# ygtxr1997/MSML

Hardware: AMD Instinct MI355X
Metric: images/sec (112x112) ires50-MSML+PartialFC training step (higher is better)
Workload: dtype bf16; 1 GPU; iresnet50-MSML (OSB r18 + FM x4) + 85742-id ArcFace PartialFC, 112x112, batch 256/GPU, fwd+bwd+clip+SGD; global_batch=256, parallelism=dp1+class-parallel head, launch=eager, weight gradients + OSB on side streams

## Files before the change

msml_amd/csrc/wgrad_halo.hip:

```cpp
#include <stdlib.h>

#include <type_traits>

#include <mutex>

#include "common.h"
#include "options.h"

typedef __attribute__((ext_vector_type(4))) short s16x4;
typedef __attribute__((ext_vector_type(8))) short s16x8;
typedef __attribute__((address_space(3))) void* lptr_t;

#define WH_OOB 0x78000000u

typedef __attribute__((ext_vector_type(4))) unsigned int wh_rsrc_t;
__device__ __forceinline__ void wh_dma16(const wh_rsrc_t& rs, unsigned int lds, unsigned int off) {
#if defined(__HIP_DEVICE_COMPILE__)
  unsigned int keep;
  asm volatile("s_mov_b32 %0, m0\n\ts_mov_b32 m0, %3\n\ts_nop 0\n\tbuffer_load_dwordx4 %1, %2, 0 offen lds\n\ts_mov_b32 m0, %0"
               : "=&s"(keep)
               : "v"(off), "s"(rs), "s"(lds)
               : "memory");
#endif
}
__device__ __forceinline__ void wh_dma_wait() {
#if defined(__HIP_DEVICE_COMPILE__)
  asm volatile("s_waitcnt vmcnt(0)" ::: "memory");
#endif
}

#define WH_MAXGROUP 8
struct WgradHaloArgs {
  const unsigned short* u[WH_MAXGROUP]; int up; unsigned int u_bytes;
  const unsigned short* v[WH_MAXGROUP]; int vp; unsigned int v_bytes;
  int N, H, W, spy, spx;
  int XH, XW;
  int nstrips, chunk;
  int zper;
  int remap;
  int pair7;
  float* ws;
  BnIn xin;
};

template <int CO, bool XF = false, bool P7 = false>
__global__ void __launch_bounds__(512) __attribute__((amdgpu_waves_per_eu(2, 2))) k_wgrad_halo(const WgradHaloArgs p) {
#if defined(__HIP_DEVICE_COMPILE__)
  constexpr int NXB = 20;
  constexpr int GU = CO / 32, NI = CO / 64, UBLK = 7 * GU, NBLK = UBLK + NXB, NISS = (NBLK + 7) / 8;
  constexpr int UB = UBLK * 1024, VB = NXB * 1024, STAGE = UB + VB;
  extern __shared__ __attribute__((aligned(16))) char smem[];
  MSML_LDS_REGION(smem, 2 * STAGE + (XF ? 3 * 64 * 4 : 0));
  const int t = threadIdx.x, lane = t & 63;
  const int wave = __builtin_amdgcn_readfirstlane(t >> 6);
  constexpr bool R9 = CO == 128;
  const int mp = R9 ? (wave & 3) : (wave & 1), nh = R9 ? (wave >> 2) : ((wave >> 1) & 1), tg = R9 ? 0 : (wave >> 2);
  int bx = blockIdx.x, by = blockIdx.y, bz = blockIdx.z;
  if (p.remap) {
    const int T = gridDim.x * gridDim.y, total = T * gridDim.z;
    const int L = bx + gridDim.x * (by + gridDim.y * bz);
    const int Lp = (L & 7) * (total >> 3) + (L >> 3);
    const int tile = Lp % T;
    bz = Lp / T;
    bx = tile % gridDim.x;
    by = tile / gridDim.x;
  }
  const int layer = __builtin_amdgcn_readfirstlane(bz / p.zper);
  const int a0 = bx * CO, b0 = by * 64, split = bz - layer * p.zper;
  const int s_begin = split * p.chunk;
  int s_end = s_begin + p.chunk;
  if (s_end > p.nstrips) s_end = p.nstrips;
  const int spi = p.spy * p.spx;

  auto make_rsrc = [](const void* ptr, unsigned int bytes) -> wh_rsrc_t {
    const unsigned long long a = (unsigned long long)ptr;
    wh_rsrc_t r;
    r[0] = __builtin_amdgcn_readfirstlane((unsigned int)a);
    r[1] = __builtin_amdgcn_readfirstlane((unsigned int)(a >> 32) & 0xffffu);
    r[2] = __builtin_amdgcn_readfirstlane(bytes);
    r[3] = 0x00020000u;
    return r;
  };
  const wh_rsrc_t rs_u = make_rsrc(p.u[layer], p.u_bytes), rs_v = make_rsrc(p.v[layer], p.v_bytes);
  const unsigned int lds0 = __builtin_amdgcn_readfirstlane((unsigned int)(size_t)(lptr_t)smem);
  auto dma = [&](const wh_rsrc_t& rs, const char* dst, unsigned int off) {
    wh_dma16(rs, lds0 + (unsigned int)__builtin_amdgcn_readfirstlane((int)(dst - smem)), off);
  };

  const int lp = lane >> 2, lc = lane & 3;
  auto issue = [&](int strip, int buf) {
    char* ub = smem + buf * STAGE;
    char* vb = ub + UB;
    if constexpr (P7) {
      const int n = 2 * strip + (lp >> 3), x = lp & 7;
      const bool img = n < p.N;
#pragma unroll
      for (int i = 0; i < NISS; i++) {
        const int blk = wave + 8 * i;
        if (blk >= NBLK) break;
        if (blk < UBLK) {
          const int j = blk / GU, g = blk % GU;
          const unsigned int off = (img & (x < 7)) ? (unsigned int)((n * 7 + j) * 7 + x) * (unsigned int)(p.up * 2) +
                                                         (unsigned int)(a0 + g * 32 + lc * 8) * 2u
                                                   : WH_OOB;
          dma(rs_u, ub + blk * 1024, off);
        } else {
          const int bb = blk - UBLK, hr = bb >> 1, g = bb & 1;
          const int y = hr - 1;
          const bool ok = img & ((unsigned)y < 7u) & (x > 0);
          const unsigned int off = ok ? (unsigned int)((n * 7 + y) * 7 + x - 1) * (unsigned int)(p.vp * 2) +
                                            (unsigned int)(b0 + g * 32 + lc * 8) * 2u
                                      : WH_OOB;
          dma(rs_v, vb + bb * 1024, off);
        }
      }
      return;
    }
    const int n = strip / spi, rem = strip - n * spi, sy = rem / p.spx;
    const int y0 = sy * 7, x0 = (rem - sy * p.spx) * 14;
#pragma unroll
    for (int i = 0; i < NISS; i++) {
      const int blk = wave + 8 * i;
      if (blk >= NBLK) break;
      if (blk < UBLK) {
        const int j = blk / GU, g = blk % GU;
        const int y = y0 + j, x = x0 + lp;
        const bool ok = (lp < 14) & (x < p.W) & (y < p.H);
        const unsigned int off = ok ? (unsigned int)((n * p.H + y) * p.W + x) * (unsigned int)(p.up * 2) +
                                          (unsigned int)(a0 + g * 32 + lc * 8) * 2u
                                    : WH_OOB;
        dma(rs_u, ub + blk * 1024, off);
      } else {
        const int bb = blk - UBLK, hr = bb >> 1, g = bb & 1;
        const int y = y0 + hr - 1, x = x0 + lp - 1;
        const bool ok = (hr < 9) & ((unsigned)y < (unsigned)p.H) & ((unsigned)x < (unsigned)p.W);
        const unsigned int off = ok ? (unsigned int)((n * p.H + y) * p.W + x) * (unsigned int)(p.vp * 2) +
                                          (unsigned int)(b0 + g * 32 + lc * 8) * 2u
                                    : WH_OOB;
        dma(rs_v, vb + bb * 1024, off);
      }
    }
  };

  float* xtab = reinterpret_cast<float*>(smem + 2 * STAGE);
  auto xform = [&](int strip, int buf) {
    const int n = strip / spi, rem = strip - n * spi, sy = rem / p.spx;
    const int y0 = sy * 7, x0 = (rem - sy * p.spx) * 14;
    char* vb = smem + buf * STAGE + UB;
    const bool has_alpha = p.xin.alpha != nullptr;
#pragma unroll
    for (int i = 0; i < NISS; i++) {
      const int blk = wave + 8 * i;
      if (blk >= NBLK) break;
      if (blk >= UBLK) {
        const int bb = blk - UBLK, hr = bb >> 1, g = bb & 1;
        const int y = y0 + hr - 1, x = x0 + lp - 1;
        if ((hr < 9) & ((unsigned)y < (unsigned)p.H) & ((unsigned)x < (unsigned)p.W))
          bn_in_chunk(vb + bb * 1024 + lane * 16, xtab, 64, g * 32 + lc * 8, has_alpha);
      }
    }
  };

  constexpr int NA = R9 ? 1 : NI, NK = R9 ? 9 : 5;
  f32x16 acc[NA][NK];
#pragma unroll
  for (int i = 0; i < NA; i++)
#pragma unroll
    for (int k = 0; k < NK; k++)
#pragma unroll
      for (int e = 0; e < 16; e++) acc[i][k][e] = 0.f;

  const int g4 = lane >> 4, i16 = lane & 15, q4 = i16 >> 2, pp = i16 & 3;
  const int px = 8 * (g4 >> 1) + q4;
  const int chan = (2 * (g4 & 1) + (pp >> 1)) * 16 + (pp & 1) * 8;
  const int aofs = mp * NA * 1024 + px * 64 + chan;
  int vlo[3], vhi[3];
#pragma unroll
  for (int s = 0; s < 3; s++) {
    const int p0 = px + s, p1 = px + 4 + s;
    vlo[s] = nh * 1024 + (p0 >> 4) * 2048 + (p0 & 15) * 64 + chan;
    vhi[s] = nh * 1024 + (p1 >> 4) * 2048 + (p1 & 15) * 64 + chan;
  }
  const int ntaps = R9 ? 9 : (tg == 0 ? 5 : 4), tap0 = tg * 5;
  int vlok[5], vhik[5];
#pragma unroll
  for (int k = 0; k < 5; k++) {
    const int tp = tap0 + k, r = tp / 3, sft = tp - r * 3;
    vlok[k] = r * 2048 + (sft == 0 ? vlo[0] : (sft == 1 ? vlo[1] : vlo[2]));
    vhik[k] = r * 2048 + (sft == 0 ? vhi[0] : (sft == 1 ? vhi[1] : vhi[2]));
  }
  typedef __attribute__((address_space(3))) s16x4* tr_ptr;
  auto tr2 = [&](const char* lo, const char* hi) -> s16x8 {
    s16x4 l = __builtin_amdgcn_ds_read_tr16_b64_v4i16((tr_ptr)(lo));
    s16x4 h = __builtin_amdgcn_ds_read_tr16_b64_v4i16((tr_ptr)(hi));
    s16x8 o;
    o[0] = l[0]; o[1] = l[1]; o[2] = l[2]; o[3] = l[3];
    o[4] = h[0]; o[5] = h[1]; o[6] = h[2]; o[7] = h[3];
    return o;
  };

  if (s_begin < s_end) issue(s_begin, 0);
  if (XF) bn_in_fill(p.xin, xtab, b0, 64, t, 512);
  wh_dma_wait();
  __syncthreads();
  if (XF) {
    if (s_begin < s_end) xform(s_begin, 0);
    __syncthreads();
  }
  int cur = 0;
  s16x8 fa[2][NA], fb5[2][5], xr[4][3];
  for (int strip = s_begin; strip < s_end; strip++) {
    if (strip + 1 < s_end) issue(strip + 1, cur ^ 1);
    const char* ub = smem + cur * STAGE + aofs;
    const char* vb = smem + cur * STAGE + UB;
    if constexpr (R9) {
      auto fetch_a = [&](int j) { fa[j & 1][0] = tr2(ub + j * (GU * 1024), ub + j * (GU * 1024) + 256); };
      auto fetch_x = [&](int row) {
#pragma unroll
        for (int sft = 0; sft < 3; sft++) xr[row & 3][sft] = tr2(vb + row * 2048 + vlo[sft], vb + row * 2048 + vhi[sft]);
      };
      fetch_a(0);
      fetch_x(0);
      fetch_x(1);
      fetch_x(2);
#pragma unroll
      for (int j = 0; j < 7; j++) {
        if (j + 1 < 7) {
          fetch_a(j + 1);
          fetch_x(j + 3);
        }
        __builtin_amdgcn_sched_barrier(0);
#pragma unroll
        for (int k = 0; k < 9; k++)
          acc[0][k] = __builtin_amdgcn_mfma_f32_32x32x16_bf16(__builtin_bit_cast(bf16x8, fa[j & 1][0]),
                                                              __builtin_bit_cast(bf16x8, xr[(j + k / 3) & 3][k % 3]),
                                                              acc[0][k], 0, 0, 0);
        __builtin_amdgcn_sched_barrier(0);
        if (XF && j == 6 && strip + 1 < s_end) {
          wh_dma_wait();
          xform(strip + 1, cur ^ 1);
        }
      }
      wh_dma_wait();
      __syncthreads();
      cur ^= 1;
      continue;
    }
    auto fetch = [&](int j, int fb) {
#pragma unroll
      for (int i = 0; i < NA; i++)
        fa[fb][i] = tr2(ub + j * (GU * 1024) + i * 1024, ub + j * (GU * 1024) + i * 1024 + 256);
#pragma unroll
      for (int k = 0; k < 5; k++)
        if (k < ntaps) fb5[fb][k] = tr2(vb + j * 2048 + vlok[k], vb + j * 2048 + vhik[k]);
    };
    fetch(0, 0);
#pragma unroll
    for (int j = 0; j < 7; j++) {
      const int fb = j & 1;
      if (j + 1 < 7) fetch(j + 1, fb ^ 1);
      __builtin_amdgcn_sched_barrier(0);
#pragma unroll
      for (int k = 0; k < 5; k++)
        if (k < ntaps) {
#pragma unroll
          for (int i = 0; i < NA; i++)
            acc[i][k] = __builtin_amdgcn_mfma_f32_32x32x16_bf16(__builtin_bit_cast(bf16x8, fa[fb][i]),
                                                                __builtin_bit_cast(bf16x8, fb5[fb][k]), acc[i][k], 0, 0, 0);
        }
      __builtin_amdgcn_sched_barrier(0);
      if (XF && j == (CO == 128 ? 6 : 2) && strip + 1 < s_end) {
        asm volatile("s_waitcnt vmcnt(0)" ::: "memory");
        xform(strip + 1, cur ^ 1);
      }
    }
    wh_dma_wait();
    __syncthreads();
    cur ^= 1;
  }

  const int h = lane >> 5, c32 = lane & 31;
  const int b = b0 + nh * 32 + c32;
#pragma unroll
  for (int i = 0; i < NA; i++)
#pragma unroll
    for (int k = 0; k < NK; k++) {
      if (k >= ntaps) continue;
#pragma unroll
      for (int e = 0; e < 16; e++) {
        const int a = a0 + (mp * NA + i) * 32 + (e & 3) + 8 * (e >> 2) + 4 * h;
        p.ws[(((long)bz * p.up + a) * 9 + tap0 + k) * p.vp + b] = acc[i][k][e];
      }
    }
#endif
}

static int wh_cus() {
  static int n = 0;
  if (n == 0) {
    int dev = 0;
    if (hipGetDevice(&dev) != hipSuccess || hipDeviceGetAttribute(&n, hipDeviceAttributeMultiprocessorCount, dev) != hipSuccess || n <= 0)
      n = 256;
  }
  return n;
}

static bool wh_wide(int up) {
  const int lim = msml_opt().wgrad_halo_wide_min;
  return up % 128 == 0 && up >= lim;
}

int msml_wgrad_halo_splits(int up, int vp, int A, int Breal, int N, int H, int W, int P, int Q, int R, int S,
                           int stride, int pad_h, int pad_w) {
  const bool off = msml_opt().no_halo_wgrad;
  if (off) return 0;
  if (R != 3 || S != 3 || stride != 1 || pad_h != 1 || pad_w != 1 || P != H || Q != W) return 0;
  if (up % 64 != 0 || vp % 64 != 0 || A != up || Breal != vp) return 0;
  const bool pair7 = H == 7 && W == 7 && !msml_opt().wgrad_halo_no_pair7;
  const long strips = pair7 ? (N + 1) / 2 : (long)N * cdiv(H, 7) * cdiv(W, 14);
  if ((long)N * H * W * 10 < strips * 112 * 7) return 0;
  if ((long)N * H * W * up * 2 >= 0x70000000L || (long)N * H * W * vp * 2 >= 0x70000000L) return 0;
  const int tiles = ((wh_wide(up) && !pair7) ? up / 128 : up / 64) * (vp / 64);
  long splits = wh_cus() / tiles;
  if (splits < 1) splits = 1;
  if (splits > strips) splits = strips;
  if (splits > 512) splits = 512;
  return (int)splits;
}

template <int CO, bool XF, bool P7 = false>
static void wh_launch(const WgradHaloArgs& a, dim3 grid, hipStream_t st) {
  const size_t lds = 2 * (7 * (CO / 32) + 10 * 2) * 1024 + (XF ? 3 * 64 * sizeof(float) : 0);
  static std::once_flag attr_once;
  std::call_once(attr_once, [&] {
    (void)hipFuncSetAttribute(reinterpret_cast<const void*>(&k_wgrad_halo<CO, XF, P7>),
                              hipFuncAttributeMaxDynamicSharedMemorySize, (int)lds);
  });
  k_wgrad_halo<CO, XF, P7><<<grid, dim3(512), lds, st>>>(a);
}

int msml_wgrad_halo_group_splits(int up, int vp, int A, int Breal, int N, int H, int W, int P, int Q, int R, int S,
                                 int stride, int pad_h, int pad_w, int group) {
  const int hs = msml_wgrad_halo_splits(up, vp, A, Breal, N, H, W, P, Q, R, S, stride, pad_h, pad_w);
  if (hs <= 0 || group < 1 || group > WH_MAXGROUP) return 0;
  const int per = hs / group;
  return per < 1 ? 0 : per;
}

bool msml_wgrad_halo_launch_group(const void* const* u, int up, const void* const* v, int vp, float* ws, int N, int H,
                                  int W, int group, int splits, hipStream_t st, const BnIn* xin) {
  const bool no_remap = msml_opt().wgrad_halo_no_remap;
  WgradHaloArgs a;
  for (int i = 0; i < WH_MAXGROUP; i++) {
    a.u[i] = (const unsigned short*)u[i < group ? i : 0];
    a.v[i] = (const unsigned short*)v[i < group ? i : 0];
  }
  a.up = up; a.u_bytes = (unsigned int)((long)N * H * W * up * 2);
  a.vp = vp; a.v_bytes = (unsigned int)((long)N * H * W * vp * 2);
  a.N = N; a.H = H; a.W = W; a.spy = cdiv(H, 7); a.spx = cdiv(W, 14);
  a.pair7 = (H == 7 && W == 7) ? 1 : 0;
  a.nstrips = a.pair7 ? (N + 1) / 2 : N * a.spy * a.spx;
  a.chunk = cdiv(a.nstrips, splits);
  a.zper = splits;
  a.ws = ws;
  a.xin = BnIn{nullptr, nullptr, nullptr};
  if (xin) a.xin = *xin;
  const int gz = group * splits;
  const int tiles = ((wh_wide(up) && !a.pair7) ? up / 128 : up / 64) * (vp / 64);
  a.remap = (!no_remap && tiles >= 4 && gz % 8 == 0) ? 1 : 0;
  if (a.pair7) {
    if (xin) return false;
    wh_launch<64, false, true>(a, dim3(up / 64, vp / 64, gz), st);
    return true;
  }
  if (wh_wide(up)) {
    if (xin) wh_launch<128, true>(a, dim3(up / 128, vp / 64, gz), st);
    else wh_launch<128, false>(a, dim3(up / 128, vp / 64, gz), st);
  } else {
    if (xin) wh_launch<64, true>(a, dim3(up / 64, vp / 64, gz), st);
    else wh_launch<64, false>(a, dim3(up / 64, vp / 64, gz), st);
  }
  return true;
}

bool msml_wgrad_halo_launch(const void* u, int up, const void* v, int vp, float* ws, int N, int H, int W,
// ... 4 lines not shown
```

msml_amd/csrc/fc_wgrad.hip:

```cpp
#include <stdlib.h>

#include <mutex>

#include "common.h"
#include "options.h"

typedef __attribute__((ext_vector_type(4))) short s16x4;
typedef __attribute__((ext_vector_type(8))) short s16x8;
typedef __attribute__((address_space(3))) void* lptr_t;

#define FCW_OOB 0x78000000u
#define FCW_NISS 7
#define FCW_MAX_TAPS 51

struct FcWgradArgs {
  const unsigned short* u; unsigned int u_bytes;
  const unsigned short* v; unsigned int v_bytes;
  int N, T, up, vp;
  float* dw;
  long row_stride;
  int boff, accumulate;
};

__global__ void __launch_bounds__(512) k_fc_wgrad(const FcWgradArgs p) {
// ... 8 lines not shown
  __amdgpu_buffer_rsrc_t rs_u = __builtin_amdgcn_make_buffer_rsrc((void*)p.u, 0, (int)p.u_bytes, 0x00020000);
  __amdgpu_buffer_rsrc_t rs_v = __builtin_amdgcn_make_buffer_rsrc((void*)p.v, 0, (int)p.v_bytes, 0x00020000);

  const int lp = lane >> 2, lc = lane & 3;
  auto issue = [&](int step, int buf) {
    char* sb = smem + buf * stage_bytes;
    const int n = step * 16 + lp;
    const bool nok = n < p.N;
#pragma unroll
    for (int i = 0; i < FCW_NISS; i++) {
      const int blk = wave + 8 * i;
      if (blk > T) {
        __builtin_amdgcn_raw_ptr_buffer_load_lds(rs_u, (lptr_t)(sb + (T + 1) * 1024), 16, FCW_OOB, 0, 0, 0);
      } else if (blk == 0) {
        const unsigned int off = nok ? (unsigned int)(n * p.up + e0) * 2u + (unsigned int)lc * 16u : FCW_OOB;
        __builtin_amdgcn_raw_ptr_buffer_load_lds(rs_u, (lptr_t)sb, 16, off, 0, 0, 0);
      } else {
        const unsigned int off = nok ? (unsigned int)((n * T + blk - 1) * p.vp + c0) * 2u + (unsigned int)lc * 16u : FCW_OOB;
        __builtin_amdgcn_raw_ptr_buffer_load_lds(rs_v, (lptr_t)(sb + blk * 1024), 16, off, 0, 0, 0);
      }
    }
  };

  f32x16 acc[FCW_NISS];
#pragma unroll
  for (int k = 0; k < FCW_NISS; k++)
#pragma unroll
    for (int e = 0; e < 16; e++) acc[k][e] = 0.f;

  const int g4 = lane >> 4, i16 = lane & 15, q4 = i16 >> 2, pp = i16 & 3;
  const int px = 8 * (g4 >> 1) + q4;
  const int chan = (2 * (g4 & 1) + (pp >> 1)) * 16 + (pp & 1) * 8;
  const int aofs = px * 64 + chan;
  typedef __attribute__((address_space(3))) s16x4* tr_ptr;
  auto tr2 = [&](const char* lo) -> s16x8 {
    s16x4 l = __builtin_amdgcn_ds_read_tr16_b64_v4i16((tr_ptr)(lo));
    s16x4 h = __builtin_amdgcn_ds_read_tr16_b64_v4i16((tr_ptr)(lo + 256));
    s16x8 o;
    o[0] = l[0]; o[1] = l[1]; o[2] = l[2]; o[3] = l[3];
    o[4] = h[0]; o[5] = h[1]; o[6] = h[2]; o[7] = h[3];
    return o;
  };
  int ntaps = 0;
#pragma unroll
  for (int k = 0; k < FCW_NISS; k++) ntaps += (wave + 8 * k < T) ? 1 : 0;

  issue(0, 0);
  if (nsteps > 1) issue(1, 1);
  int cur = 0, nxt = 2;
  for (int step = 0; step < nsteps; step++) {
    if (step + 1 < nsteps) asm volatile("s_waitcnt vmcnt(%0)" ::"n"(FCW_NISS) : "memory");
    else asm volatile("s_waitcnt vmcnt(0)" ::: "memory");
    __builtin_amdgcn_s_barrier();
    if (step + 2 < nsteps) issue(step + 2, nxt);
    const char* sb = smem + cur * stage_bytes + aofs;
    const s16x8 fa = tr2(sb);
#pragma unroll
    for (int k = 0; k < FCW_NISS; k++)
      if (k < ntaps) {
        const s16x8 fb = tr2(sb + (1 + wave + 8 * k) * 1024);
        acc[k] = __builtin_amdgcn_mfma_f32_32x32x16_bf16(__builtin_bit_cast(bf16x8, fa), __builtin_bit_cast(bf16x8, fb),
                                                         acc[k], 0, 0, 0);
      }
    cur = cur == 2 ? 0 : cur + 1;
    nxt = nxt == 2 ? 0 : nxt + 1;
  }
  __syncthreads();

  float* tile = reinterpret_cast<float*>(smem);
  MSML_LDS_REGION(smem, 3 * stage_bytes);
  MSML_LDS_REGION(tile, 16 * 32 * T * 4);
  const int RL = 32 * T, RL4 = RL >> 2;
  const int h = lane >> 5, b = lane & 31;
  for (int hf = 0; hf < 2; hf++) {
#pragma unroll
    for (int k = 0; k < FCW_NISS; k++) {
      if (k >= ntaps) continue;
      const int tp = wave + 8 * k;
#pragma unroll
      for (int e8 = 0; e8 < 8; e8++) {
        const int arow = (e8 & 3) + 8 * (e8 >> 2) + 4 * h;
        tile[arow * RL + b * T + tp] = hf ? acc[k][8 + e8] : acc[k][e8];
      }
    }
    __syncthreads();
    for (int idx = t; idx < 16 * RL4; idx += 512) {
      const int row = idx / RL4, c4 = idx - row * RL4;
      float* g = p.dw + (long)(e0 + 16 * hf + row) * p.row_stride + (long)(p.boff + c0) * T + c4 * 4;
      f32x4 o = *reinterpret_cast<const f32x4*>(tile + row * RL + c4 * 4);
      if (p.accumulate) {
        const f32x4 old = *reinterpret_cast<const f32x4*>(g);
        o[0] += old[0]; o[1] += old[1]; o[2] += old[2]; o[3] += old[3];
      }
      *reinterpret_cast<f32x4*>(g) = o;
    }
    __syncthreads();
  }
#endif
}

int msml_fc_wgrad_launch(const void* u, int up, const void* v, int vp, float* dw, int A, int Breal, int Btot, int boff,
                         int N, int H, int W, int P, int Q, int R, int S, int stride, int pad_h, int pad_w,
                         int accumulate, hipStream_t st) {
  const bool off = msml_opt().no_fc_wgrad;
  const int T = R * S;
  if (off || P != 1 || Q != 1 || R != H || S != W || pad_h != 0 || pad_w != 0 || stride != 1) return 0;
  if (T < 2 || T > FCW_MAX_TAPS || up % 32 || vp % 32 || A != up || Breal != vp || N < 16) return 0;
  if (boff % 4 || ((long)Btot * T) % 4 || ((size_t)dw % 16)) return 0;
  if ((long)N * T * vp * 2 >= 0x70000000L || (long)N * up * 2 >= 0x70000000L) return 0;
  FcWgradArgs a;
  a.u = (const unsigned short*)u; a.u_bytes = (unsigned int)((long)N * up * 2);
  a.v = (const unsigned short*)v; a.v_bytes = (unsigned int)((long)N * T * vp * 2);
  a.N = N; a.T = T; a.up = up; a.vp = vp;
  a.dw = dw; a.row_stride = (long)Btot * T; a.boff = boff; a.accumulate = accumulate;
  const int lds = 3 * (T + 2) * 1024;
  static std::once_flag once;
// ... 8 lines not shown
```

msml_amd/csrc/wgrad_fast.hip:

```cpp
#include <stdlib.h>

#include "common.h"

typedef __attribute__((ext_vector_type(4))) short s16x4;
typedef __attribute__((ext_vector_type(8))) short s16x8;
typedef __attribute__((address_space(3))) void* lptr_t;

#define OOB_OFFSET 0x7ffffff0u

#define WF_MAXGROUP 8
struct WgradFastArgs {
  const unsigned short* u[WF_MAXGROUP]; int up; unsigned int u_bytes;
  const unsigned short* v[WF_MAXGROUP]; int vp; unsigned int v_bytes;
  int zper;
  int N, H, W, P, Q, R, S, stride, pad_h, pad_w;
  float* ws;
  int arows;
  long Mpix;
  int chunk;
  float rcp_pq, rcp_q;
  float* dw[WF_MAXGROUP];
  int direct;
  int A, Breal, Btot, boff, accumulate;
};
// ... 55 lines not shown
    const unsigned int ubase = in ? (unsigned int)m * (unsigned int)(p.up * 2) : OOB_OFFSET;
    unsigned int vbase[NTW];
#pragma unroll
    for (int tw = 0; tw < NTW; tw++) {
      const int tp = tap0 + tw;
      const int r = tp / p.S, s = tp - r * p.S;
      const int iy = iy0 + r, ix = ix0 + s;
      const bool vok = in & ((unsigned)iy < (unsigned)p.H) & ((unsigned)ix < (unsigned)p.W);
      vbase[tw] = vok ? (unsigned int)((n * p.H + iy) * p.W + ix) * (unsigned int)(p.vp * 2) : OOB_OFFSET;
    }
    char* ub = smem + buf * STAGE + wave * (GA * 1024);
    char* vb = smem + buf * STAGE + UBYTES + wave * (GB * 1024);
    unsigned int ou[GA], ov[GB];
#pragma unroll
    for (int g = 0; g < GA; g++) ou[g] = (ubase | uoffc[g]) >= OOB_OFFSET ? OOB_OFFSET : ubase + uoffc[g];
#pragma unroll
    for (int g = 0; g < GB; g++)
      ov[g] = (vbase[g / GPT] | voffc[g]) >= OOB_OFFSET ? OOB_OFFSET : vbase[g / GPT] + voffc[g];
#pragma unroll
    for (int g = 0; g < GA; g++)
      __builtin_amdgcn_raw_ptr_buffer_load_lds(rs_u, (lptr_t)(ub + g * 1024), 16, ou[g], 0, 0, 0);
#pragma unroll
    for (int g = 0; g < GB; g++)
      __builtin_amdgcn_raw_ptr_buffer_load_lds(rs_v, (lptr_t)(vb + g * 1024), 16, ov[g], 0, 0, 0);
  };

  f32x16 acc[TM][TN];
#pragma unroll
  for (int i = 0; i < TM; i++)
#pragma unroll
    for (int j = 0; j < TN; j++)
#pragma unroll
      for (int e = 0; e < 16; e++) acc[i][j][e] = 0.f;

  const int wm = wave >> 1, wn = wave & 1;
  const int arow0 = wm * (BA / 2), bcol0 = wn * (BB / 2);
  const int g4 = lane >> 4, i16 = lane & 15, q4 = i16 >> 2, pp = i16 & 3;
  const int frag = (8 * (g4 >> 1) + q4) * 64 + (2 * (g4 & 1) + (pp >> 1)) * 16 + (pp & 1) * 8;
  const int aofs = (arow0 / 32) * 1024 + frag, bofs = (bcol0 / 32) * 1024 + frag;
  typedef __attribute__((address_space(3))) s16x4* tr_ptr;
  auto trf = [&](const char* base) -> s16x8 {
    s16x4 lo = __builtin_amdgcn_ds_read_tr16_b64_v4i16((tr_ptr)(base));
    s16x4 hi = __builtin_amdgcn_ds_read_tr16_b64_v4i16((tr_ptr)(base + 256));
    s16x8 o;
    o[0] = lo[0]; o[1] = lo[1]; o[2] = lo[2]; o[3] = lo[3];
    o[4] = hi[0]; o[5] = hi[1]; o[6] = hi[2]; o[7] = hi[3];
    return o;
  };

  if (nstages > 0) gissue(0, 0);
  __syncthreads();
  int cur = 0;
  for (int st = 0; st < nstages; st++) {
    if (st + 1 < nstages) gissue(st + 1, cur ^ 1);
    const char* ub = smem + cur * STAGE + aofs;
    const char* vb = smem + cur * STAGE + UBYTES + bofs;
    s16x8 a[2][TM], b[2][TN];
#pragma unroll
    for (int i = 0; i < TM; i++) a[0][i] = trf(ub + i * 1024);
#pragma unroll
    for (int j = 0; j < TN; j++) b[0][j] = trf(vb + j * 1024);
#pragma unroll
    for (int kk = 0; kk < 4; kk++) {
      const int cb = kk & 1, nb = cb ^ 1;
      if (kk + 1 < 4) {
#pragma unroll
        for (int i = 0; i < TM; i++) a[nb][i] = trf(ub + (kk + 1) * (GA * 1024) + i * 1024);
#pragma unroll
        for (int j = 0; j < TN; j++) b[nb][j] = trf(vb + (kk + 1) * (GB * 1024) + j * 1024);
      }
      __builtin_amdgcn_sched_barrier(0);
#pragma unroll
      for (int i = 0; i < TM; i++)
#pragma unroll
        for (int j = 0; j < TN; j++)
          acc[i][j] = __builtin_amdgcn_mfma_f32_32x32x16_bf16(
              __builtin_bit_cast(bf16x8, a[cb][i]), __builtin_bit_cast(bf16x8, b[cb][j]), acc[i][j], 0, 0, 0);
      __builtin_amdgcn_sched_barrier(0);
    }
    __syncthreads();
    cur ^= 1;
  }

  const int h = lane >> 5, c32 = lane & 31;
#pragma unroll
  for (int i = 0; i < TM; i++)
#pragma unroll
    for (int j = 0; j < TN; j++) {
      const int col = bcol0 + 32 * j + c32;
      const int tap = tap0 + col / (GPT * 32);
      const int b = b0 + col % (GPT * 32);
#pragma unroll
      for (int e = 0; e < 16; e++) {
        const int a = a0 + arow0 + 32 * i + (e & 3) + 8 * (e >> 2) + 4 * h;
        if (p.direct) {
          if (a < p.A && b < p.Breal && tap < taps) {
            float* dwl = p.dw[layer];
            const long o = ((long)a * p.Btot + p.boff + b) * taps + tap;
            dwl[o] = p.accumulate ? dwl[o] + acc[i][j][e] : acc[i][j][e];
          }
        } else if (a < p.arows && b < p.vp && tap < taps) {
          p.ws[(((long)blockIdx.z * p.arows + a) * taps + tap) * p.vp + b] = acc[i][j][e];
        }
      }
    }
#endif
}



bool msml_wgrad_fast_launch_group(const void* const* u, int up, const void* const* v, int vp, float* ws, int N, int H,
                                  int W, int P, int Q, int R, int S, int stride, int pad_h, int pad_w, int ba, int bb,
                                  int ntw, int group, int splits, int chunk, hipStream_t st, float* const* dw_direct,
                                  int A, int Breal, int Btot, int boff, int accumulate) {
  const long ub = (long)N * P * Q * up * 2, vb = (long)N * H * W * vp * 2;
  if (ub >= 0x7fffff00L || vb >= 0x7fffff00L || group < 1 || group > WF_MAXGROUP) return false;
  WgradFastArgs a;
  for (int i = 0; i < WF_MAXGROUP; i++) {
    a.u[i] = (const unsigned short*)u[i < group ? i : 0];
    a.v[i] = (const unsigned short*)v[i < group ? i : 0];
    a.dw[i] = dw_direct ? dw_direct[i < group ? i : 0] : nullptr;
  }
  a.up = up; a.u_bytes = (unsigned int)ub;
  a.vp = vp; a.v_bytes = (unsigned int)vb;
  a.zper = splits;
  a.N = N; a.H = H; a.W = W; a.P = P; a.Q = Q; a.R = R; a.S = S;
  a.stride = stride; a.pad_h = pad_h; a.pad_w = pad_w;
  a.ws = ws; a.arows = up;
  a.Mpix = (long)N * P * Q;
  a.chunk = chunk;
  a.rcp_pq = 1.0f / (float)(P * Q);
  a.rcp_q = 1.0f / (float)Q;
// ... 28 lines not shown
```

msml_amd/csrc/wgrad_n32.hip:

```cpp
#include <stdlib.h>

#include <mutex>

#include "common.h"
#include "options.h"

typedef __attribute__((ext_vector_type(4))) short s16x4;
typedef __attribute__((ext_vector_type(8))) short s16x8;
typedef __attribute__((address_space(3))) void* lptr_t;

#define WN_OOB 0x78000000u

struct WgradN32Args {
  const unsigned short* u; unsigned int u_bytes;
  const unsigned short* v; unsigned int v_bytes;
  int N, P, Q, H, W, spy, spx;
  int nstrips, chunk;
  float* ws;
};

template <int R, int STRIDE>
__global__ void __launch_bounds__(512) k_wgrad_n32(const WgradN32Args p) {
#if defined(__HIP_DEVICE_COMPILE__)
  constexpr int TAPS = R * R, SR = 4, VR = STRIDE * SR + R - STRIDE, NPL = STRIDE;
// ... 39 lines not shown
        if (STRIDE == 2) {
          x = 2 * x0 - 1 + 2 * jj + plane;
          y = 2 * y0 - 1 + vrow;
          ok = jj <= 16;
        } else {
          x = x0 - 1 + jj;
          y = y0 - 1 + vrow;
          ok = jj < 18;
        }
        ok = ok & ((unsigned)x < (unsigned)p.W) & ((unsigned)y < (unsigned)p.H);
        const unsigned int off = ok ? (unsigned int)((n * p.H + y) * p.W + x) * 64u + (unsigned int)lc * 16u : WN_OOB;
        __builtin_amdgcn_raw_ptr_buffer_load_lds(rs_v, (lptr_t)(vb + bb * 1024), 16, off, 0, 0, 0);
      }
    }
  };

  f32x16 acc[2];
#pragma unroll
  for (int k = 0; k < 2; k++)
#pragma unroll
    for (int e = 0; e < 16; e++) acc[k][e] = 0.f;

  const int g4 = lane >> 4, i16 = lane & 15, q4 = i16 >> 2, pp = i16 & 3;
  const int px = 8 * (g4 >> 1) + q4;
  const int chan = (2 * (g4 & 1) + (pp >> 1)) * 16 + (pp & 1) * 8;
  const int aofs = px * 64 + chan;
  const int ntaps = (wave + 8 < TAPS) ? 2 : (wave < TAPS ? 1 : 0);
  int vofs[2], vrow0[2];
#pragma unroll
  for (int k = 0; k < 2; k++) {
    const int tp = wave + 8 * k < TAPS ? wave + 8 * k : 0;
    const int r = tp / R, s = tp - r * R;
    const int plane = STRIDE == 2 ? (s & 1) : 0, shift = STRIDE == 2 ? (s >> 1) : s;
    vrow0[k] = r;
    vofs[k] = plane * 2048 + (px + shift) * 64 + chan;
  }
  typedef __attribute__((address_space(3))) s16x4* tr_ptr;
  auto tr2 = [&](const char* lo) -> s16x8 {
    s16x4 l = __builtin_amdgcn_ds_read_tr16_b64_v4i16((tr_ptr)(lo));
    s16x4 h = __builtin_amdgcn_ds_read_tr16_b64_v4i16((tr_ptr)(lo + 256));
    s16x8 o;
    o[0] = l[0]; o[1] = l[1]; o[2] = l[2]; o[3] = l[3];
    o[4] = h[0]; o[5] = h[1]; o[6] = h[2]; o[7] = h[3];
    return o;
  };

  if (s_begin < s_end) issue(s_begin, 0);
  if (s_begin + 1 < s_end) issue(s_begin + 1, 1);
  int cur = 0, nxt = 2;
  for (int strip = s_begin; strip < s_end; strip++) {
    if (strip + 1 < s_end) asm volatile("s_waitcnt vmcnt(%0)" ::"n"(NISS) : "memory");
    else asm volatile("s_waitcnt vmcnt(0)" ::: "memory");
    __builtin_amdgcn_s_barrier();
    if (strip + 2 < s_end) issue(strip + 2, nxt);
    const char* ub = smem + cur * STAGE + aofs;
    const char* vb = smem + cur * STAGE + UB;
#pragma unroll
    for (int j = 0; j < SR; j++) {
      const s16x8 fa = tr2(ub + j * 1024);
#pragma unroll
      for (int k = 0; k < 2; k++)
        if (k < ntaps) {
          const s16x8 fb = tr2(vb + (STRIDE * j + vrow0[k]) * (NPL * 2048) + vofs[k]);
          acc[k] = __builtin_amdgcn_mfma_f32_32x32x16_bf16(__builtin_bit_cast(bf16x8, fa), __builtin_bit_cast(bf16x8, fb),
                                                           acc[k], 0, 0, 0);
        }
    }
    cur = cur == 2 ? 0 : cur + 1;
    nxt = nxt == 2 ? 0 : nxt + 1;
  }

  const int h = lane >> 5, b = lane & 31;
#pragma unroll
  for (int k = 0; k < 2; k++) {
    if (k >= ntaps) continue;
    const int tp = wave + 8 * k;
#pragma unroll
    for (int e = 0; e < 16; e++) {
      const int a = (e & 3) + 8 * (e >> 2) + 4 * h;
      p.ws[(((long)split * 32 + a) * TAPS + tp) * 32 + b] = acc[k][e];
    }
  }
#endif
}

static int wn_cus() {
  static int n = 0;
  if (n == 0) {
    int dev = 0;
    if (hipGetDevice(&dev) != hipSuccess || hipDeviceGetAttribute(&n, hipDeviceAttributeMultiprocessorCount, dev) != hipSuccess || n <= 0)
      n = 256;
  }
  return n;
}

int msml_wgrad_n32_splits(int up, int vp, int N, int H, int W, int P, int Q, int R, int S, int stride, int pad_h,
                          int pad_w) {
  const bool off = msml_opt().no_n32_wgrad;
  if (off || up != 32 || vp != 32 || R != S || pad_h != 1 || pad_w != 1) return 0;
  const bool d4 = R == 4 && stride == 2 && H == 2 * P && W == 2 * Q;
  const bool c3 = R == 3 && stride == 1 && H == P && W == Q;
  if (!d4 && !c3) return 0;
  if (P < 14 || Q < 14) return 0;
  if ((long)N * H * W * 64 >= 0x70000000L) return 0;
  const long strips = (long)N * cdiv(P, 4) * cdiv(Q, 16);
  long splits = 2L * wn_cus();
  if (d4) splits = wn_cus();
  if (splits > strips) splits = strips;
  if (splits > 512) splits = 512;
  return (int)splits;
}

template <int R, int STRIDE>
static void wn_launch(const WgradN32Args& a, int splits, hipStream_t st) {
  constexpr int VR = STRIDE * 4 + R - STRIDE;
  const size_t lds = 3 * (4 * 1024 + VR * STRIDE * 2048 + 1024);
  static std::once_flag attr_once;
  std::call_once(attr_once, [&] {
    (void)hipFuncSetAttribute(reinterpret_cast<const void*>(&k_wgrad_n32<R, STRIDE>),
                              hipFuncAttributeMaxDynamicSharedMemorySize, (int)lds);
// ... 40 lines not shown
  int t_end = t_begin + p.chunk;
  if (t_end > p.ntiles) t_end = p.ntiles;

  __amdgpu_buffer_rsrc_t rs_u = __builtin_amdgcn_make_buffer_rsrc((void*)p.u, 0, (int)p.u_bytes, 0x00020000);
  __amdgpu_buffer_rsrc_t rs_v = __builtin_amdgcn_make_buffer_rsrc((void*)p.v, 0, (int)p.v_bytes, 0x00020000);
  const int lp = lane >> 2, lc = lane & 3;
  auto issue = [&](int tile, int buf) {
    const int n = tile / p.tiles_per_img, b0 = (tile - n * p.tiles_per_img) * B;
    char* ub = smem + buf * STAGE;
    char* vb = ub + UB;
    for (int blk = wave; blk < NBLK; blk += 8) {
      if (blk < UBLK) {
        const int q = blk * 16 + lp, a = q / B, b = b0 + (q - a * B);
        const bool ok = b < L;
        const int y = p.vertical ? a : b, x = p.vertical ? b : a;
        const unsigned int off = ok ? (unsigned int)((n * L + y) * L + x) * 64u + (unsigned int)lc * 16u : WN_OOB;
        __builtin_amdgcn_raw_ptr_buffer_load_lds(rs_u, (lptr_t)(ub + blk * 1024), 16, off, 0, 0, 0);
      } else {
        const int bb = blk - UBLK, hf = bb / VBLK, j = bb - hf * VBLK;
        const int q = j * 16 + lp, a = q / B - 3, b = b0 + (q - (q / B) * B);
        const bool ok = (q < nreg) & ((unsigned)a < (unsigned)L) & (b < L);
        const int y = p.vertical ? a : b, x = p.vertical ? b : a;
        const unsigned int off = ok ? (unsigned int)((n * L + y) * L + x) * (unsigned int)(VP * 2) + (unsigned int)(hf * 64 + lc * 16)
                                    : WN_OOB;
        __builtin_amdgcn_raw_ptr_buffer_load_lds(rs_v, (lptr_t)(vb + bb * 1024), 16, off, 0, 0, 0);
      }
    }
  };

  f32x16 acc[NH];
#pragma unroll
  for (int k = 0; k < NH; k++)
#pragma unroll
    for (int e = 0; e < 16; e++) acc[k][e] = 0.f;
  const int g4 = lane >> 4, i16 = lane & 15, q4 = i16 >> 2, pp = i16 & 3;
  const int px = 8 * (g4 >> 1) + q4;
  const int chan = (2 * (g4 & 1) + (pp >> 1)) * 16 + (pp & 1) * 8;
  const int aofs = px * 64 + chan;
  const int vofs = (wave < 7 ? wave : 0) * B * 64 + px * 64 + chan;
  typedef __attribute__((address_space(3))) s16x4* tr_ptr;
  auto tr2 = [&](const char* lo) -> s16x8 {
    s16x4 l = __builtin_amdgcn_ds_read_tr16_b64_v4i16((tr_ptr)(lo));
    s16x4 h = __builtin_amdgcn_ds_read_tr16_b64_v4i16((tr_ptr)(lo + 256));
    s16x8 o;
    o[0] = l[0]; o[1] = l[1]; o[2] = l[2]; o[3] = l[3];
    o[4] = h[0]; o[5] = h[1]; o[6] = h[2]; o[7] = h[3];
    return o;
  };

  if (t_begin < t_end) issue(t_begin, 0);
  __syncthreads();
  int cur = 0;
  for (int tile = t_begin; tile < t_end; tile++) {
    if (tile + 1 < t_end) issue(tile + 1, cur ^ 1);
    if (wave < 7) {
      const char* ub = smem + cur * STAGE + aofs;
      const char* vb = smem + cur * STAGE + UB + vofs;
#pragma unroll
      for (int j = 0; j < UBLK; j++) {
        const s16x8 fa = tr2(ub + j * 1024);
#pragma unroll
        for (int k = 0; k < NH; k++) {
          const s16x8 fb = tr2(vb + k * (VBLK * 1024) + j * 1024);
          acc[k] = __builtin_amdgcn_mfma_f32_32x32x16_bf16(__builtin_bit_cast(bf16x8, fa), __builtin_bit_cast(bf16x8, fb),
                                                           acc[k], 0, 0, 0);
        }
      }
    }
    __syncthreads();
    cur ^= 1;
  }
  if (wave < 7) {
    const int h = lane >> 5, b = lane & 31;
#pragma unroll
    for (int k = 0; k < NH; k++)
#pragma unroll
      for (int e = 0; e < 16; e++) {
        const int a = (e & 3) + 8 * (e >> 2) + 4 * h;
        p.ws[(((long)split * 32 + a) * 7 + wave) * VP + k * 32 + b] = acc[k][e];
      }
  }
#endif
}

int msml_wgrad_line_splits(int up, int vp, int N, int H, int W, int P, int Q, int R, int S, int stride, int pad_h,
                           int pad_w) {
  const bool off = msml_opt().no_n32_wgrad;
  if (off || up != 32 || (vp != 32 && vp != 64) || stride != 1) return 0;
  if (!((R == 7 && S == 1 && pad_h == 3 && pad_w == 0) || (R == 1 && S == 7 && pad_h == 0 && pad_w == 3))) return 0;
  if (H != W || P != H || Q != W || !(H == 56 || H == 28)) return 0;
  if ((long)N * H * W * vp * 2 >= 0x70000000L) return 0;
  const long tiles = (long)N * cdiv(H, 224 / H);
  long splits = (vp == 32 ? 2L : 1L) * wn_cus();
  if (splits > tiles) splits = tiles;
  if (splits > 512) splits = 512;
  return (int)splits;
}

template <int VP>
static void wl_launch(const WgradLineArgs& a, int splits, hipStream_t st) {
  const size_t lds = 2 * (size_t)(14 + (VP / 32) * 18) * 1024;
  static std::once_flag attr_once;
  std::call_once(attr_once, [&] {
    (void)hipFuncSetAttribute(reinterpret_cast<const void*>(&k_wgrad_line<VP>), hipFuncAttributeMaxDynamicSharedMemorySize,
                              (int)lds);
  });
  k_wgrad_line<VP><<<dim3(splits), dim3(512), lds, st>>>(a);
}

bool msml_wgrad_line_launch(const void* u, const void* v, int vp, float* ws, int N, int H, int R, int splits,
                            hipStream_t st) {
  WgradLineArgs a;
  a.u = (const unsigned short*)u; a.u_bytes = (unsigned int)((long)N * H * H * 64);
  a.v = (const unsigned short*)v; a.v_bytes = (unsigned int)((long)N * H * H * vp * 2);
  a.N = N; a.L = H; a.B = 224 / H;
  a.tiles_per_img = cdiv(H, a.B);
  a.ntiles = N * a.tiles_per_img;
  a.chunk = cdiv(a.ntiles, splits);
  a.vertical = R == 7 ? 1 : 0;
  a.ws = ws;
  if (vp == 64) wl_launch<64>(a, splits, st);
// ... 4 lines not shown
```

Baseline: 9011 images/sec.

## Triple-buffer halo wgrad strips and pipeline LDS fetches across strip boundaries

Moves the halo weight-gradient kernel from double to triple LDS buffering. Each strip's DMA is now issued two strips ahead and split across wave groups mid-strip, and the first fragments of the next strip are fetched during the last row of the current one. Strip index decoding is replaced by incremental position advancing, which drops per-strip integer divides. The goal is to hide global-to-LDS latency and the barrier stalls at strip ends. In exchange it uses 1.5x the LDS per block, which could hurt occupancy or fail the waves-per-EU target, and the rotating register slots add risk.

```diff
diff --git a/msml_amd/csrc/wgrad_halo.hip b/msml_amd/csrc/wgrad_halo.hip
--- a/msml_amd/csrc/wgrad_halo.hip
+++ b/msml_amd/csrc/wgrad_halo.hip
@@ -28,6 +28,14 @@
   asm volatile("s_waitcnt vmcnt(0)" ::: "memory");
 #endif
 }
+
+#define WH_JB 3
+__host__ __device__ constexpr int wh_aslot(int j) { return j == 0 ? 2 : ((j - 1) & 1); }
+template <bool SIX>
+__host__ __device__ constexpr int wh_xslot(int r) {
+  return SIX ? (r < 5 ? r : (r == 5 ? 0 : (r == 6 ? 5 : r - 4))) : (r < 8 ? (r & 3) : 4);
+}
+struct WhPos { int n, sy, sx; };
 
 #define WH_MAXGROUP 8
 struct WgradHaloArgs {
@@ -50,7 +58,7 @@
   constexpr int GU = CO / 32, NI = CO / 64, UBLK = 7 * GU, NBLK = UBLK + NXB, NISS = (NBLK + 7) / 8;
   constexpr int UB = UBLK * 1024, VB = NXB * 1024, STAGE = UB + VB;
   extern __shared__ __attribute__((aligned(16))) char smem[];
-  MSML_LDS_REGION(smem, 2 * STAGE + (XF ? 3 * 64 * 4 : 0));
+  MSML_LDS_REGION(smem, 3 * STAGE + (XF ? 3 * 64 * 4 : 0));
   const int t = threadIdx.x, lane = t & 63;
   const int wave = __builtin_amdgcn_readfirstlane(t >> 6);
   constexpr bool R9 = CO == 128;
@@ -70,7 +78,23 @@
   const int s_begin = split * p.chunk;
   int s_end = s_begin + p.chunk;
   if (s_end > p.nstrips) s_end = p.nstrips;
-  const int spi = p.spy * p.spx;
+  auto decode = [&](int strip) -> WhPos {
+    if constexpr (P7) return WhPos{2 * strip, 0, 0};
+    const int spi = p.spy * p.spx;
+    const int n = strip / spi, rem = strip - n * spi, sy = rem / p.spx;
+    return WhPos{n, sy, rem - sy * p.spx};
+  };
+  auto advance = [&](WhPos& q) {
+    if constexpr (P7) {
+      q.n += 2;
+    } else if (++q.sx == p.spx) {
+      q.sx = 0;
+      if (++q.sy == p.spy) {
+        q.sy = 0;
+        q.n++;
+      }
+    }
+  };
 
   auto make_rsrc = [](const void* ptr, unsigned int bytes) -> wh_rsrc_t {
     const unsigned long long a = (unsigned long long)ptr;
@@ -88,11 +112,11 @@
   };
 
   const int lp = lane >> 2, lc = lane & 3;
-  auto issue = [&](int strip, int buf) {
+  auto issue = [&](const WhPos& q, int buf) {
     char* ub = smem + buf * STAGE;
     char* vb = ub + UB;
     if constexpr (P7) {
-      const int n = 2 * strip + (lp >> 3), x = lp & 7;
+      const int n = q.n + (lp >> 3), x = lp & 7;
       const bool img = n < p.N;
 #pragma unroll
       for (int i = 0; i < NISS; i++) {
@@ -116,8 +140,7 @@
       }
       return;
     }
-    const int n = strip / spi, rem = strip - n * spi, sy = rem / p.spx;
-    const int y0 = sy * 7, x0 = (rem - sy * p.spx) * 14;
+    const int n = q.n, y0 = q.sy * 7, x0 = q.sx * 14;
 #pragma unroll
     for (int i = 0; i < NISS; i++) {
       const int blk = wave + 8 * i;
@@ -142,10 +165,9 @@
     }
   };
 
-  float* xtab = reinterpret_cast<float*>(smem + 2 * STAGE);
-  auto xform = [&](int strip, int buf) {
-    const int n = strip / spi, rem = strip - n * spi, sy = rem / p.spx;
-    const int y0 = sy * 7, x0 = (rem - sy * p.spx) * 14;
+  float* xtab = reinterpret_cast<float*>(smem + 3 * STAGE);
+  auto xform = [&](const WhPos& q, int buf) {
+    const int y0 = q.sy * 7, x0 = q.sx * 14;
     char* vb = smem + buf * STAGE + UB;
     const bool has_alpha = p.xin.alpha != nullptr;
 #pragma unroll
@@ -199,84 +221,151 @@
     return o;
   };
 
-  if (s_begin < s_end) issue(s_begin, 0);
+  WhPos qi = decode(s_begin), qx = qi;
+  if (s_begin < s_end) {
+    issue(qi, 0);
+    advance(qi);
+  }
   if (XF) bn_in_fill(p.xin, xtab, b0, 64, t, 512);
   wh_dma_wait();
+  if (s_begin + 1 < s_end) {
+    issue(qi, 1);
+    advance(qi);
+  }
   __syncthreads();
   if (XF) {
-    if (s_begin < s_end) xform(s_begin, 0);
+    if (s_begin < s_end) {
+      xform(qx, 0);
+      advance(qx);
+    }
     __syncthreads();
   }
   int cur = 0;
-  s16x8 fa[2][NA], fb5[2][5], xr[4][3];
-  for (int strip = s_begin; strip < s_end; strip++) {
-    if (strip + 1 < s_end) issue(strip + 1, cur ^ 1);
-    const char* ub = smem + cur * STAGE + aofs;
-    const char* vb = smem + cur * STAGE + UB;
-    if constexpr (R9) {
-      auto fetch_a = [&](int j) { fa[j & 1][0] = tr2(ub + j * (GU * 1024), ub + j * (GU * 1024) + 256); };
-      auto fetch_x = [&](int row) {
-#pragma unroll
-        for (int sft = 0; sft < 3; sft++) xr[row & 3][sft] = tr2(vb + row * 2048 + vlo[sft], vb + row * 2048 + vhi[sft]);
-      };
-      fetch_a(0);
-      fetch_x(0);
-      fetch_x(1);
-      fetch_x(2);
+  auto mid_strip = [&](int strip, int nx1) {
+    if (strip + 1 >= s_end) return;
+    wh_dma_wait();
+    if (XF) {
+      xform(qx, nx1);
+      advance(qx);
+    }
+    __syncthreads();
+  };
+  auto request = [&](int j, int strip, int nx2) {
+    if (j != WH_JB + 1 + (wave >> 2)) return;
+    if (strip + 2 < s_end) {
+      issue(qi, nx2);
+      advance(qi);
+    }
+  };
+  constexpr bool SIX = !XF;
+  s16x8 fa[3][NA], fb5[3][5], xr[SIX ? 6 : 5][3];
+  if constexpr (R9) {
+    auto fetch_a = [&](const char* ub, int j) {
+      fa[wh_aslot(j)][0] = tr2(ub + j * (GU * 1024), ub + j * (GU * 1024) + 256);
+    };
+    auto fetch_x = [&](const char* vb, int row) {
+#pragma unroll
+      for (int sft = 0; sft < 3; sft++)
+        xr[wh_xslot<SIX>(row)][sft] = tr2(vb + row * 2048 + vlo[sft], vb + row * 2048 + vhi[sft]);
+    };
+    auto mfmas = [&](int j, int k0, int k1) {
+#pragma unroll
+      for (int k = k0; k < k1; k++)
+        acc[0][k] = __builtin_amdgcn_mfma_f32_32x32x16_bf16(__builtin_bit_cast(bf16x8, fa[wh_aslot(j)][0]),
+                                                            __builtin_bit_cast(bf16x8, xr[wh_xslot<SIX>(j + k / 3)][k % 3]),
+                                                            acc[0][k], 0, 0, 0);
+    };
+    fetch_a(smem + aofs, 0);
+    fetch_x(smem + UB, 0);
+    if (SIX) {
+      fetch_x(smem + UB, 1);
+      fetch_x(smem + UB, 2);
+    }
+    for (int strip = s_begin; strip < s_end; strip++) {
+      const int nx1 = cur == 2 ? 0 : cur + 1, nx2 = nx1 == 2 ? 0 : nx1 + 1;
+      const char* ub = smem + cur * STAGE + aofs;
+      const char* vb = smem + cur * STAGE + UB;
 #pragma unroll
       for (int j = 0; j < 7; j++) {
+        constexpr int KF = 3;
+        if (j == 0) {
+          __builtin_amdgcn_sched_barrier(0);
+          mfmas(0, 0, KF);
+          __builtin_amdgcn_sched_barrier(0);
+          if (!SIX) {
+            fetch_x(vb, 1);
+            fetch_x(vb, 2);
+          }
+        }
         if (j + 1 < 7) {
-          fetch_a(j + 1);
-          fetch_x(j + 3);
+          fetch_a(ub, j + 1);
+          fetch_x(vb, j + 3);
+          __builtin_amdgcn_sched_barrier(0);
+          mfmas(j, j == 0 ? KF : 0, 9);
+          __builtin_amdgcn_sched_barrier(0);
+        } else {
+          const char* ubn = smem + nx1 * STAGE + aofs;
+          const char* vbn = smem + nx1 * STAGE + UB;
+          fetch_a(ubn, 0);
+          fetch_x(vbn, 0);
+          __builtin_amdgcn_sched_barrier(0);
+          mfmas(j, 0, 3);
+          __builtin_amdgcn_sched_barrier(0);
+          if (SIX) {
+            fetch_x(vbn, 1);
+            fetch_x(vbn, 2);
+          }
+          __builtin_amdgcn_sched_barrier(0);
+          mfmas(j, 3, 9);
+          __builtin_amdgcn_sched_barrier(0);
         }
-        __builtin_amdgcn_sched_barrier(0);
-#pragma unroll
-        for (int k = 0; k < 9; k++)
-          acc[0][k] = __builtin_amdgcn_mfma_f32_32x32x16_bf16(__builtin_bit_cast(bf16x8, fa[j & 1][0]),
-                                                              __builtin_bit_cast(bf16x8, xr[(j + k / 3) & 3][k % 3]),
-                                                              acc[0][k], 0, 0, 0);
-        __builtin_amdgcn_sched_barrier(0);
-        if (XF && j == 6 && strip + 1 < s_end) {
-          wh_dma_wait();
-          xform(strip + 1, cur ^ 1);
+        if (j == WH_JB) mid_strip(strip, nx1);
+        if (j == WH_JB + 1 || j == WH_JB + 2) request(j, strip, nx2);
+      }
+      cur = nx1;
+    }
+  } else {
+    auto fetch = [&](int buf, int j) {
+      const char* ub = smem + buf * STAGE + aofs;
+      const char* vb = smem + buf * STAGE + UB;
+#pragma unroll
+      for (int i = 0; i < NA; i++)
+        fa[wh_aslot(j)][i] = tr2(ub + j * (GU * 1024) + i * 1024, ub + j * (GU * 1024) + i * 1024 + 256);
+#pragma unroll
+      for (int k = 0; k < 5; k++)
+        if (k < ntaps) fb5[wh_aslot(j)][k] = tr2(vb + j * 2048 + vlok[k], vb + j * 2048 + vhik[k]);
+    };
+    auto mfmas = [&](int j, int k0, int k1) {
+#pragma unroll
+      for (int k = k0; k < k1; k++)
+        if (k < ntaps) {
+#pragma unroll
+          for (int i = 0; i < NA; i++)
+            acc[i][k] = __builtin_amdgcn_mfma_f32_32x32x16_bf16(__builtin_bit_cast(bf16x8, fa[wh_aslot(j)][i]),
+                                                                __builtin_bit_cast(bf16x8, fb5[wh_aslot(j)][k]),
+                                                                acc[i][k], 0, 0, 0);
         }
-      }
-      wh_dma_wait();
-      __syncthreads();
-      cur ^= 1;
-      continue;
-    }
-    auto fetch = [&](int j, int fb) {
-#pragma unroll
-      for (int i = 0; i < NA; i++)
-        fa[fb][i] = tr2(ub + j * (GU * 1024) + i * 1024, ub + j * (GU * 1024) + i * 1024 + 256);
-#pragma unroll
-      for (int k = 0; k < 5; k++)
-        if (k < ntaps) fb5[fb][k] = tr2(vb + j * 2048 + vlok[k], vb + j * 2048 + vhik[k]);
     };
     fetch(0, 0);
-#pragma unroll
-    for (int j = 0; j < 7; j++) {
-      const int fb = j & 1;
-      if (j + 1 < 7) fetch(j + 1, fb ^ 1);
-      __builtin_amdgcn_sched_barrier(0);
-#pragma unroll
-      for (int k = 0; k < 5; k++)
-        if (k < ntaps) {
-#pragma unroll
-          for (int i = 0; i < NA; i++)
-            acc[i][k] = __builtin_amdgcn_mfma_f32_32x32x16_bf16(__builtin_bit_cast(bf16x8, fa[fb][i]),
-                                                                __builtin_bit_cast(bf16x8, fb5[fb][k]), acc[i][k], 0, 0, 0);
+    for (int strip = s_begin; strip < s_end; strip++) {
+      const int nx1 = cur == 2 ? 0 : cur + 1, nx2 = nx1 == 2 ? 0 : nx1 + 1;
+#pragma unroll
+      for (int j = 0; j < 7; j++) {
+        if (j == 0) {
+          __builtin_amdgcn_sched_barrier(0);
+          mfmas(0, 0, 1);
+          __builtin_amdgcn_sched_barrier(0);
         }
-      __builtin_amdgcn_sched_barrier(0);
-      if (XF && j == (CO == 128 ? 6 : 2) && strip + 1 < s_end) {
-        asm volatile("s_waitcnt vmcnt(0)" ::: "memory");
-        xform(strip + 1, cur ^ 1);
-      }
-    }
-    wh_dma_wait();
-    __syncthreads();
-    cur ^= 1;
+        if (j + 1 < 7) fetch(cur, j + 1);
+        else fetch(nx1, 0);
+        __builtin_amdgcn_sched_barrier(0);
+        mfmas(j, j == 0 ? 1 : 0, 5);
+        __builtin_amdgcn_sched_barrier(0);
+        if (j == WH_JB) mid_strip(strip, nx1);
+        if (j == WH_JB + 1 || j == WH_JB + 2) request(j, strip, nx2);
+      }
+      cur = nx1;
+    }
   }
 
   const int h = lane >> 5, c32 = lane & 31;
@@ -330,7 +419,7 @@
 
 template <int CO, bool XF, bool P7 = false>
 static void wh_launch(const WgradHaloArgs& a, dim3 grid, hipStream_t st) {
-  const size_t lds = 2 * (7 * (CO / 32) + 10 * 2) * 1024 + (XF ? 3 * 64 * sizeof(float) : 0);
+  const size_t lds = 3 * (7 * (CO / 32) + 10 * 2) * 1024 + (XF ? 3 * 64 * sizeof(float) : 0);
   static std::once_flag attr_once;
   std::call_once(attr_once, [&] {
     (void)hipFuncSetAttribute(reinterpret_cast<const void*>(&k_wgrad_halo<CO, XF, P7>),
```

Result: no change. 9042 images/sec, median of 3 (+0.3%).

## Issue next-stage global loads after LDS fragment reads, before MFMA block

Applied to the files above, without the earlier changes.

In the FC, fast and n32 weight-gradient kernels, the main loop now reads all LDS fragments for the current stage into registers first. The async global-to-LDS loads for the next stage are issued only after that, fenced with sched_barrier, and the MFMA chain runs last. The goal is to stop the buffer_load_lds traffic from competing with the ds_read_tr fragment reads and to let the loads overlap the MFMA run. The cost is more live VGPRs, since whole stages of fragments are held at once, which could raise register pressure or lower occupancy. The HOLD/LEAD split in the line kernel is there to limit that pressure.

```diff
diff --git a/msml_amd/csrc/fc_wgrad.hip b/msml_amd/csrc/fc_wgrad.hip
--- a/msml_amd/csrc/fc_wgrad.hip
+++ b/msml_amd/csrc/fc_wgrad.hip
@@ -84,16 +84,21 @@
     if (step + 1 < nsteps) asm volatile("s_waitcnt vmcnt(%0)" ::"n"(FCW_NISS) : "memory");
     else asm volatile("s_waitcnt vmcnt(0)" ::: "memory");
     __builtin_amdgcn_s_barrier();
-    if (step + 2 < nsteps) issue(step + 2, nxt);
     const char* sb = smem + cur * stage_bytes + aofs;
     const s16x8 fa = tr2(sb);
+    s16x8 fb[FCW_NISS];
 #pragma unroll
     for (int k = 0; k < FCW_NISS; k++)
-      if (k < ntaps) {
-        const s16x8 fb = tr2(sb + (1 + wave + 8 * k) * 1024);
-        acc[k] = __builtin_amdgcn_mfma_f32_32x32x16_bf16(__builtin_bit_cast(bf16x8, fa), __builtin_bit_cast(bf16x8, fb),
+      if (k < ntaps) fb[k] = tr2(sb + (1 + wave + 8 * k) * 1024);
+    __builtin_amdgcn_sched_barrier(0);
+    if (step + 2 < nsteps) issue(step + 2, nxt);
+    __builtin_amdgcn_sched_barrier(0);
+#pragma unroll
+    for (int k = 0; k < FCW_NISS; k++)
+      if (k < ntaps)
+        acc[k] = __builtin_amdgcn_mfma_f32_32x32x16_bf16(__builtin_bit_cast(bf16x8, fa), __builtin_bit_cast(bf16x8, fb[k]),
                                                          acc[k], 0, 0, 0);
-      }
+    __builtin_amdgcn_sched_barrier(0);
     cur = cur == 2 ? 0 : cur + 1;
     nxt = nxt == 2 ? 0 : nxt + 1;
   }
diff --git a/msml_amd/csrc/wgrad_fast.hip b/msml_amd/csrc/wgrad_fast.hip
--- a/msml_amd/csrc/wgrad_fast.hip
+++ b/msml_amd/csrc/wgrad_fast.hip
@@ -131,32 +131,28 @@
   __syncthreads();
   int cur = 0;
   for (int st = 0; st < nstages; st++) {
-    if (st + 1 < nstages) gissue(st + 1, cur ^ 1);
     const char* ub = smem + cur * STAGE + aofs;
     const char* vb = smem + cur * STAGE + UBYTES + bofs;
-    s16x8 a[2][TM], b[2][TN];
-#pragma unroll
-    for (int i = 0; i < TM; i++) a[0][i] = trf(ub + i * 1024);
-#pragma unroll
-    for (int j = 0; j < TN; j++) b[0][j] = trf(vb + j * 1024);
+    s16x8 a[4][TM], b[4][TN];
 #pragma unroll
     for (int kk = 0; kk < 4; kk++) {
-      const int cb = kk & 1, nb = cb ^ 1;
-      if (kk + 1 < 4) {
-#pragma unroll
-        for (int i = 0; i < TM; i++) a[nb][i] = trf(ub + (kk + 1) * (GA * 1024) + i * 1024);
-#pragma unroll
-        for (int j = 0; j < TN; j++) b[nb][j] = trf(vb + (kk + 1) * (GB * 1024) + j * 1024);
-      }
-      __builtin_amdgcn_sched_barrier(0);
+#pragma unroll
+      for (int i = 0; i < TM; i++) a[kk][i] = trf(ub + kk * (GA * 1024) + i * 1024);
+#pragma unroll
+      for (int j = 0; j < TN; j++) b[kk][j] = trf(vb + kk * (GB * 1024) + j * 1024);
+    }
+    __builtin_amdgcn_sched_barrier(0);
+    if (st + 1 < nstages) gissue(st + 1, cur ^ 1);
+    __builtin_amdgcn_sched_barrier(0);
+#pragma unroll
+    for (int kk = 0; kk < 4; kk++)
 #pragma unroll
       for (int i = 0; i < TM; i++)
 #pragma unroll
         for (int j = 0; j < TN; j++)
           acc[i][j] = __builtin_amdgcn_mfma_f32_32x32x16_bf16(
-              __builtin_bit_cast(bf16x8, a[cb][i]), __builtin_bit_cast(bf16x8, b[cb][j]), acc[i][j], 0, 0, 0);
-      __builtin_amdgcn_sched_barrier(0);
-    }
+              __builtin_bit_cast(bf16x8, a[kk][i]), __builtin_bit_cast(bf16x8, b[kk][j]), acc[i][j], 0, 0, 0);
+    __builtin_amdgcn_sched_barrier(0);
     __syncthreads();
     cur ^= 1;
   }
diff --git a/msml_amd/csrc/wgrad_n32.hip b/msml_amd/csrc/wgrad_n32.hip
--- a/msml_amd/csrc/wgrad_n32.hip
+++ b/msml_amd/csrc/wgrad_n32.hip
@@ -115,20 +115,27 @@
     if (strip + 1 < s_end) asm volatile("s_waitcnt vmcnt(%0)" ::"n"(NISS) : "memory");
     else asm volatile("s_waitcnt vmcnt(0)" ::: "memory");
     __builtin_amdgcn_s_barrier();
-    if (strip + 2 < s_end) issue(strip + 2, nxt);
     const char* ub = smem + cur * STAGE + aofs;
     const char* vb = smem + cur * STAGE + UB;
+    s16x8 fa[SR], fb[SR][2];
 #pragma unroll
     for (int j = 0; j < SR; j++) {
-      const s16x8 fa = tr2(ub + j * 1024);
+      fa[j] = tr2(ub + j * 1024);
 #pragma unroll
       for (int k = 0; k < 2; k++)
-        if (k < ntaps) {
-          const s16x8 fb = tr2(vb + (STRIDE * j + vrow0[k]) * (NPL * 2048) + vofs[k]);
-          acc[k] = __builtin_amdgcn_mfma_f32_32x32x16_bf16(__builtin_bit_cast(bf16x8, fa), __builtin_bit_cast(bf16x8, fb),
-                                                           acc[k], 0, 0, 0);
-        }
-    }
+        if (k < ntaps) fb[j][k] = tr2(vb + (STRIDE * j + vrow0[k]) * (NPL * 2048) + vofs[k]);
+    }
+    __builtin_amdgcn_sched_barrier(0);
+    if (strip + 2 < s_end) issue(strip + 2, nxt);
+    __builtin_amdgcn_sched_barrier(0);
+#pragma unroll
+    for (int j = 0; j < SR; j++)
+#pragma unroll
+      for (int k = 0; k < 2; k++)
+        if (k < ntaps)
+          acc[k] = __builtin_amdgcn_mfma_f32_32x32x16_bf16(__builtin_bit_cast(bf16x8, fa[j]),
+                                                           __builtin_bit_cast(bf16x8, fb[j][k]), acc[k], 0, 0, 0);
+    __builtin_amdgcn_sched_barrier(0);
     cur = cur == 2 ? 0 : cur + 1;
     nxt = nxt == 2 ? 0 : nxt + 1;
   }
@@ -275,21 +282,40 @@
   __syncthreads();
   int cur = 0;
   for (int tile = t_begin; tile < t_end; tile++) {
-    if (tile + 1 < t_end) issue(tile + 1, cur ^ 1);
+    constexpr int HOLD = VP == 64 ? UBLK : 8, LEAD = UBLK - HOLD;
+    s16x8 fa[HOLD], fb[HOLD][NH];
     if (wave < 7) {
       const char* ub = smem + cur * STAGE + aofs;
       const char* vb = smem + cur * STAGE + UB + vofs;
 #pragma unroll
-      for (int j = 0; j < UBLK; j++) {
-        const s16x8 fa = tr2(ub + j * 1024);
+      for (int j = 0; j < LEAD; j++) {
+        const s16x8 f = tr2(ub + j * 1024);
 #pragma unroll
         for (int k = 0; k < NH; k++) {
-          const s16x8 fb = tr2(vb + k * (VBLK * 1024) + j * 1024);
-          acc[k] = __builtin_amdgcn_mfma_f32_32x32x16_bf16(__builtin_bit_cast(bf16x8, fa), __builtin_bit_cast(bf16x8, fb),
+          const s16x8 g = tr2(vb + k * (VBLK * 1024) + j * 1024);
+          acc[k] = __builtin_amdgcn_mfma_f32_32x32x16_bf16(__builtin_bit_cast(bf16x8, f), __builtin_bit_cast(bf16x8, g),
                                                            acc[k], 0, 0, 0);
         }
       }
-    }
+#pragma unroll
+      for (int j = 0; j < HOLD; j++) {
+        fa[j] = tr2(ub + (LEAD + j) * 1024);
+#pragma unroll
+        for (int k = 0; k < NH; k++) fb[j][k] = tr2(vb + k * (VBLK * 1024) + (LEAD + j) * 1024);
+      }
+    }
+    __builtin_amdgcn_sched_barrier(0);
+    if (tile + 1 < t_end) issue(tile + 1, cur ^ 1);
+    __builtin_amdgcn_sched_barrier(0);
+    if (wave < 7) {
+#pragma unroll
+      for (int j = 0; j < HOLD; j++)
+#pragma unroll
+        for (int k = 0; k < NH; k++)
+          acc[k] = __builtin_amdgcn_mfma_f32_32x32x16_bf16(__builtin_bit_cast(bf16x8, fa[j]),
+                                                           __builtin_bit_cast(bf16x8, fb[j][k]), acc[k], 0, 0, 0);
+    }
+    __builtin_amdgcn_sched_barrier(0);
     __syncthreads();
     cur ^= 1;
   }
```

Measured after the change: 9138 images/sec before, 8840 images/sec after. -3.3%, worse.
